# felipescoelho/w-ofdm-optimization

Measured on AMD Instinct MI355X. Metric: OFDM symbols/sec (whole node) + BER vs reference, N=256 16-QAM, higher is better.
Workload: dtype f32

## Files before the change

### w-ofdm-optimization_amd/csrc/wofdm_abi.hip

```cpp
#include "../../include/wofdm.h"
#include "wofdm_kernel.h"

#include <algorithm>
#include <cmath>
#include <complex>
#include <cstdarg>
#include <cstdio>
#include <cstdlib>
#include <cstring>
#include <mutex>
#include <utility>
#include <vector>

namespace {

thread_local char g_err[512] = "";
thread_local float g_papr_ms = 0.f;
thread_local float g_rxprof_ms = 0.f;

int fail(int code, const char *fmt, ...)
{
    va_list ap;
    va_start(ap, fmt);
    vsnprintf(g_err, sizeof g_err, fmt, ap);
// ... 28 lines not shown
        return fail(WOFDM_E_UNSUPPORTED, "n_taps=%d not in [1,%d]", c->n_taps, WOFDM_MAX_TAPS);
    if (c->cp < 0 || c->cs < 0 || c->tail_tx < 0 || c->tail_rx < 0 || (c->tail_rx & 1) ||
        c->prefix_rm < 0 || c->circ_shift < 0 || c->circ_shift >= N)
        return fail(WOFDM_E_INVALID, "negative length, odd tail_rx or circ_shift >= n_fft");
    if (c->cp > N || c->cs > N || c->tail_rx > N)
        return fail(WOFDM_E_INVALID, "cp, cs and tail_rx must not exceed n_fft");
    if (c->n_channels < 1 || c->n_snr < 1 || c->n_window_pairs < 1)
        return fail(WOFDM_E_INVALID, "n_channels, n_snr, n_window_pairs must be >= 1");
    g->N = N; g->k = c->bits_per_sc; g->S = c->syms_per_frame;
    g->mu = c->cp; g->rho = c->cs; g->beta = c->tail_tx; g->delta = c->tail_rx;
    g->gamma = c->prefix_rm; g->kappa = c->circ_shift; g->L = c->n_taps;
    g->P = N + g->mu + g->rho; g->B = g->P - g->beta; g->T = g->beta + g->S * g->B;
    g->NL = c->noise_before_truncate ? g->T + g->L - 1 : g->S * g->B;
    if (2 * g->beta > g->P) return fail(WOFDM_E_INVALID, "2*tail_tx exceeds the symbol length");
    if (g->B != N + g->delta + g->gamma)
        return fail(WOFDM_E_INVALID, "n_fft+cp+cs-tail_tx (%d) != n_fft+tail_rx+prefix_rm (%d)",
                    g->B, N + g->delta + g->gamma);
    if (g->mu + g->rho > wofdm_cpcs_max(N) || g->beta > 16 || g->delta > 64)
        return fail(WOFDM_E_UNSUPPORTED, "kernel limits: cp+cs <= %d, tail_tx <= 16, tail_rx <= 64",
                    wofdm_cpcs_max(N));
    if (g->B > 64 * wofdm_rb(N))
        return fail(WOFDM_E_UNSUPPORTED, "cp+cs-tail_tx=%d exceeds the 64 samples the kernel's "
                    "FIR tiling allows", g->B - N);
    const uint64_t cells = (uint64_t)c->n_channels * c->n_snr * c->n_window_pairs;
    if (cells >= (1u << 28)) return fail(WOFDM_E_UNSUPPORTED, "more than 2^28 cells");
    return WOFDM_OK;
}

}

struct wofdm_plan {
    int device = 0;
    wofdm_cfg cfg{};
    geom g{};
    uint32_t n_cells = 0;
    float *d_wtx = nullptr, *d_wrx = nullptr, *d_nlin = nullptr;
    float2 *d_h = nullptr;
    int *d_geo = nullptr;
    float2 *d_nscr = nullptr;
    uint64_t nscr_elems = 0;
    wofdm_kparams base{};
    wofdm_kernel_fn fn[4] = {nullptr, nullptr, nullptr, nullptr};
    int var = WOFDM_VAR_PLAIN;
    bool has_alloc = false, has_mask = false;
    bool force_direct_mask = false;
    bool fir_valu = false;
    bool dft_valu = false;
    int max_spw = 0;
    uint32_t *d_amask = nullptr;
    float2 *d_tmask = nullptr;
    float2 *d_tspec = nullptr;
    float *d_tspec4 = nullptr;
    unsigned *d_status = nullptr;
    uint4 *d_fira = nullptr;
    float firm_sx = 1.f, firm_sh = 1.f;
    uint4 *d_dftc = nullptr;
    float *d_rxs = nullptr;
#ifdef WOFDM_AUDIT
    uint32_t *audit = nullptr;
    uint32_t audit_items = 0;
#endif
    int occ = 1, cus = 1, layout = 1;
    hipEvent_t ev0 = nullptr, ev1 = nullptr;
};

namespace {

size_t wofdm_amask_words(int N)
{
    const size_t NQ = (size_t)N / 4;
    return N == 256 ? 2 * NQ + 256 : NQ + (NQ > 256 ? NQ : 256);
}

int configure(wofdm_plan *pl)
{
    const geom &g = pl->g;
    const bool fft_ok = g.N <= WOFDM_TXFFT_MAX_N && 3 * g.P - 2 <= WOFDM_TXFFT_LEN && !pl->force_direct_mask;
    const int var = pl->has_mask ? (fft_ok ? WOFDM_VAR_TXFFT : WOFDM_VAR_TXMASK)
                                 : (pl->has_alloc ? WOFDM_VAR_ALLOC : WOFDM_VAR_PLAIN);
    const bool masked = var == WOFDM_VAR_TXMASK || var == WOFDM_VAR_TXFFT;
    const bool firm = !pl->fir_valu;
    const bool mdft = !pl->dft_valu;
    int layout = masked ? wofdm_pick_layout_masked(g.N, g.B, firm) : wofdm_pick_layout(g.N, g.S, g.B, true, firm, mdft);
    if (var == WOFDM_VAR_TXFFT && g.N == 256 && layout == 9 && mdft && WOFDM_TXFFT_LEN == 1024) layout = 15;
    if (pl->max_spw > 0 && wofdm_layout_info(layout, g.N).spw > pl->max_spw)
        layout = (pl->max_spw == 1) ? 1 : wofdm_pick_layout(g.N, g.S, g.B, false);
#ifndef WOFDM_DEV_LDS_PAD
#define WOFDM_DEV_LDS_PAD 0
#endif
    const auto lds_of = [&](int lay) {
        return wofdm_lds_bytes(g.N, g.T, lay, g.S, g.B)
               + (var == WOFDM_VAR_TXMASK ? wofdm_txmask_lds_bytes(g.N) : 0u)
               + (var == WOFDM_VAR_TXFFT && lay != 15 ? wofdm_txfft_lds_bytes() : 0u) + (unsigned)(WOFDM_DEV_LDS_PAD);
    };
    if (!masked && layout != 1 && wofdm_layout_info(layout, g.N).fir == WOFDM_FIR_ONE && lds_of(layout) > 160u * 1024u
        && lds_of(1) <= 160u * 1024u)
        layout = 1;
    const unsigned lds = lds_of(layout);
    if (lds > 160u * 1024u)
        return fail(WOFDM_E_UNSUPPORTED, "frame needs %u bytes of LDS (160 KiB per workgroup)", lds);
    wofdm_kernel_fn fn[4];
    for (int m = 0; m < 4; ++m) {
        fn[m] = wofdm_select_kernel(g.N, g.k, layout, m, var);
        if (!fn[m])
            return fail(WOFDM_E_UNSUPPORTED, "no kernel for n_fft=%d bits_per_sc=%d variant %d%s", g.N, g.k,
                        var, masked ? " (the Tx mask needs n_fft <= 512)" : "");
// ... 53 lines not shown
        const double ang = M_PI * (double)(((long long)k * k) % (2LL * L)) / (double)L;
        c[(size_t)k] = cplx(std::cos(ang), std::sin(ang));
    }
    for (int k = 0; k < L; ++k) a[(size_t)k] = (double)mask[k] * c[(size_t)k];
    b[0] = std::conj(c[0]);
    for (int k = 1; k < L; ++k) b[(size_t)k] = b[Mb - (size_t)k] = std::conj(c[(size_t)k]);
    fft_pow2(a, -1);
    fft_pow2(b, -1);
    for (size_t i = 0; i < Mb; ++i) a[i] *= b[i];
    fft_pow2(a, +1);
    std::vector<cplx> g((size_t)L);
    for (int n = 0; n < L; ++n) g[(size_t)n] = a[(size_t)n] * c[(size_t)n] / ((double)Mb * (double)L);
    return g;
}

void mask_fastconv_spectrum(const float *mask, int L, int MF, float2 *spec)
{
    const int P = (L + 1) / 2, G = 3 * P - 2;
    const std::vector<cplx> g = idft_any(mask, L);
    std::vector<cplx> gt((size_t)MF, cplx(0.0, 0.0));
    for (int t = 0; t < G && t < MF; ++t) gt[(size_t)t] = g[(size_t)(((t - (P - 1)) % L + L) % L)];
    fft_pow2(gt, -1);
    for (int f = 0; f < MF; ++f)
        spec[f] = make_float2((float)(gt[(size_t)f].real() / MF), (float)(gt[(size_t)f].imag() / MF));
}

std::mutex g_gate_mu;
hipEvent_t g_gate_last[64] = {};

int launch(wofdm_plan *pl, int mode, wofdm_kparams &kp, uint64_t total_items, int force_grid,
           hipStream_t stream)
{
    wofdm_kernel_fn fn = pl->fn[mode];
    if (!fn) return fail(WOFDM_E_UNSUPPORTED, "no kernel for n_fft=%d", pl->g.N);
    if (total_items == 0) return WOFDM_OK;
    uint64_t grid = (uint64_t)pl->cus * (uint64_t)pl->occ;
#ifdef WOFDM_DEV_OCC
    grid = (uint64_t)pl->cus * (uint64_t)(WOFDM_DEV_OCC);
#endif
    if (grid > total_items) grid = total_items;
    if (force_grid > 0) grid = (uint64_t)force_grid;
    const size_t row = wofdm_noise_scratch_len(pl->g.N, pl->layout);
    if (row && grid * row > pl->nscr_elems) {
        HIP_TRY(hipDeviceSynchronize());
        if (pl->d_nscr) (void)hipFree(pl->d_nscr);
        pl->d_nscr = nullptr; pl->nscr_elems = 0;
        HIP_TRY(hipMalloc(&pl->d_nscr, grid * row * sizeof(float2)));
        pl->nscr_elems = grid * row;
    }
    kp.noise_scratch = pl->d_nscr;
    kp.status = pl->d_status;
    kp.dftc = pl->d_dftc;
    kp.rx_scale = pl->d_rxs;
    kp.items_q = total_items / grid;
    kp.items_r = total_items % grid;
    kp.lds_bytes = pl->base.lds_bytes;
    float2 *tm = pl->var == WOFDM_VAR_TXFFT ? (pl->layout == 15 ? reinterpret_cast<float2 *>(pl->d_tspec4) : pl->d_tspec) : pl->d_tmask;
    kp.tx_scale = pl->base.tx_scale;
    kp.dump_unscale_tx = pl->base.dump_unscale_tx;
    kp.dump_unscale_rx = pl->base.dump_unscale_rx;
#ifdef WOFDM_AUDIT
    kp.audit = pl->audit; kp.audit_items = pl->audit_items;
#endif
#ifdef WOFDM_DELAY
    {
        const char *dp = std::getenv("WOFDM_DELAY_POINT"), *dw = std::getenv("WOFDM_DELAY_WAVES"), *dn = std::getenv("WOFDM_DELAY_LEN");
        kp.delay_point = dp ? (uint32_t)std::strtoul(dp, nullptr, 0) : 0;
        kp.delay_waves = dw ? (uint32_t)std::strtoul(dw, nullptr, 0) : 0;
        kp.delay_len = dn ? (uint32_t)std::strtoul(dn, nullptr, 0) : 8;
    }
#endif
    void *args[] = {&kp, &pl->d_wtx, &pl->d_wrx, &pl->d_h, &pl->d_nlin, &pl->d_geo, &pl->d_amask, &tm,
                    &pl->d_fira};
    {
        std::lock_guard<std::mutex> lock(g_gate_mu);
        hipEvent_t *last = g_gate_last;
        const int dev = pl->device & 63;
        if (last[dev]) HIP_TRY(hipStreamWaitEvent(stream, last[dev], 0));
        else HIP_TRY(hipEventCreateWithFlags(&last[dev], hipEventDisableTiming));
        HIP_TRY(hipLaunchKernel(reinterpret_cast<const void *>(fn), dim3((unsigned)grid),
                                dim3(64u * (unsigned)wofdm_waves(pl->layout, pl->g.N, pl->g.S, pl->g.B)), args, kp.lds_bytes, stream));
        HIP_TRY(hipEventRecord(last[dev], stream));
    }
    return WOFDM_OK;
}

int check_status(wofdm_plan *pl)
{
    unsigned st = 0;
    HIP_TRY(hipMemcpy(&st, pl->d_status, sizeof st, hipMemcpyDeviceToHost));
    if (st != 0)
        return fail(WOFDM_E_HIP, "kernel status 0x%x: a wave timed out waiting for its workgroup "
                    "(results must not be used)", st);
    return WOFDM_OK;
}

int check_launch_args(wofdm_plan *pl, uint64_t frames_per_cell)
{
    if (!pl) return fail(WOFDM_E_INVALID, "plan is NULL");
    if (frames_per_cell > (1ull << 40)) return fail(WOFDM_E_INVALID, "frames_per_cell too large");
    return WOFDM_OK;
}


template <typename T> struct dev_buf {
    T *p = nullptr;
    dev_buf() = default;
    dev_buf(dev_buf &&o) noexcept : p(o.p) { o.p = nullptr; }
    ~dev_buf() { if (p) (void)hipFree(p); }
    bool alloc(size_t count) { return hipMalloc(&p, count * sizeof(T)) == hipSuccess; }
    bool upload(const void *host, size_t count) { return hipMemcpy(p, host, count * sizeof(T), hipMemcpyHostToDevice) == hipSuccess; }
    operator T *() const { return p; }
};

int use_device(int device)
{
    int ndev = 0;
    HIP_TRY(hipGetDeviceCount(&ndev));
    if (device < 0 || device >= ndev)
        return fail(WOFDM_E_HIP, "device %d not available (%d visible); there is no CPU fallback", device, ndev);
    HIP_TRY(hipSetDevice(device));
    return WOFDM_OK;
}

std::vector<float2> pack_taps(const wofdm_cfg *cfg, const geom &g, const float *h)
{
    std::vector<float2> hp((size_t)cfg->n_channels * WOFDM_LT, make_float2(0.f, 0.f));
    for (int c = 0; c < cfg->n_channels; ++c)
        for (int l = 0; l < g.L; ++l)
            hp[(size_t)c * WOFDM_LT + l] = make_float2(h[2 * ((size_t)c * g.L + l)], h[2 * ((size_t)c * g.L + l) + 1]);
    return hp;
}
// ... 134 lines not shown
            const double rms = (double)pl->firm_sx * (double)pl->firm_sh * std::sqrt(e * (1.0 + (double)nlin[i]) / (double)g.N)
                               * std::fmax(wmax, 1e-30);
            if (rms > 0.0 && std::isfinite(rms))
                rxs[(size_t)i * cfg->n_channels + c] = (float)std::exp2(std::round(4.0 - std::log2(rms)));
        }

#define PLAN_TRY(expr)                                                                        \
    do {                                                                                      \
        hipError_t e_ = (expr);                                                               \
        if (e_ != hipSuccess) {                                                               \
            wofdm_plan_destroy(pl);                                                           \
            return fail(e_ == hipErrorOutOfMemory ? WOFDM_E_NOMEM : WOFDM_E_HIP, "%s: %s",    \
                        #expr, hipGetErrorString(e_));                                        \
        }                                                                                     \
    } while (0)

    PLAN_TRY(hipMalloc(&pl->d_wtx, n_wtx * sizeof(float)));
    PLAN_TRY(hipMalloc(&pl->d_wrx, n_wrx * sizeof(float)));
    PLAN_TRY(hipMalloc(&pl->d_h, hp.size() * sizeof(float2)));
    PLAN_TRY(hipMalloc(&pl->d_nlin, nlin.size() * sizeof(float)));
    PLAN_TRY(hipMemcpy(pl->d_wtx, w_tx, n_wtx * sizeof(float), hipMemcpyHostToDevice));
    PLAN_TRY(hipMemcpy(pl->d_wrx, w_rx, n_wrx * sizeof(float), hipMemcpyHostToDevice));
    PLAN_TRY(hipMemcpy(pl->d_h, hp.data(), hp.size() * sizeof(float2), hipMemcpyHostToDevice));
    PLAN_TRY(hipMemcpy(pl->d_nlin, nlin.data(), nlin.size() * sizeof(float), hipMemcpyHostToDevice));
    PLAN_TRY(hipMalloc(&pl->d_fira, fira.size() * sizeof(_Float16)));
    PLAN_TRY(hipMemcpy(pl->d_fira, fira.data(), fira.size() * sizeof(_Float16), hipMemcpyHostToDevice));
    PLAN_TRY(hipMalloc(&pl->d_dftc, dftc.size() * sizeof(uint32_t)));
    PLAN_TRY(hipMemcpy(pl->d_dftc, dftc.data(), dftc.size() * sizeof(uint32_t), hipMemcpyHostToDevice));
    PLAN_TRY(hipMalloc(&pl->d_rxs, rxs.size() * sizeof(float)));
    PLAN_TRY(hipMemcpy(pl->d_rxs, rxs.data(), rxs.size() * sizeof(float), hipMemcpyHostToDevice));
    PLAN_TRY(hipEventCreate(&pl->ev0));
    PLAN_TRY(hipEventCreate(&pl->ev1));

    int geo[WOFDM_G_COUNT];
    geo[WOFDM_G_S] = g.S; geo[WOFDM_G_MU] = g.mu; geo[WOFDM_G_RHO] = g.rho; geo[WOFDM_G_BETA] = g.beta;
    geo[WOFDM_G_DELTA] = g.delta; geo[WOFDM_G_GAMMA] = g.gamma; geo[WOFDM_G_KAPPA] = g.kappa;
    geo[WOFDM_G_L] = g.L; geo[WOFDM_G_P] = g.P; geo[WOFDM_G_B] = g.B; geo[WOFDM_G_T] = g.T;
    geo[WOFDM_G_NL] = g.NL; geo[WOFDM_G_NSNR] = cfg->n_snr; geo[WOFDM_G_NCH] = cfg->n_channels;
    geo[WOFDM_G_FBUF] = 0;
    geo[WOFDM_G_NACT] = g.N;
    geo[WOFDM_G_SPWR] = 0;
    PLAN_TRY(hipMalloc(&pl->d_geo, sizeof geo));
    PLAN_TRY(hipMemcpy(pl->d_geo, geo, sizeof geo, hipMemcpyHostToDevice));

    wofdm_kparams &kp = pl->base;
    kp.n_cells = pl->n_cells; kp.first_cell = 0; kp.inject_base_cell = 0;
    kp.seed_lo = (uint32_t)cfg->seed; kp.seed_hi = (uint32_t)(cfg->seed >> 32);

    hipDeviceProp_t prop;
    PLAN_TRY(hipGetDeviceProperties(&prop, device));
    pl->cus = prop.multiProcessorCount;
    PLAN_TRY(hipMalloc(&pl->d_status, sizeof(unsigned)));
    PLAN_TRY(hipMemset(pl->d_status, 0, sizeof(unsigned)));
    if ((rc = configure(pl)) != WOFDM_OK) {
        wofdm_plan_destroy(pl);
        return rc;
    }
    const int occ = pl->occ;
    if (const size_t row = wofdm_noise_scratch_len(g.N, pl->layout)) {
        pl->nscr_elems = (uint64_t)pl->cus * (uint64_t)occ * row;
        PLAN_TRY(hipMalloc(&pl->d_nscr, pl->nscr_elems * sizeof(float2)));
        PLAN_TRY(hipMemset(pl->d_nscr, 0, pl->nscr_elems * sizeof(float2)));
        PLAN_TRY(hipDeviceSynchronize());
    }
#undef PLAN_TRY
    *out = pl;
    return WOFDM_OK;
}

int wofdm_plan_destroy(wofdm_plan *pl)
{
    if (!pl) return WOFDM_OK;
    (void)hipSetDevice(pl->device);
    if (pl->d_wtx) (void)hipFree(pl->d_wtx);
    if (pl->d_wrx) (void)hipFree(pl->d_wrx);
    if (pl->d_h) (void)hipFree(pl->d_h);
    if (pl->d_nlin) (void)hipFree(pl->d_nlin);
    if (pl->d_geo) (void)hipFree(pl->d_geo);
    if (pl->d_nscr) (void)hipFree(pl->d_nscr);
    if (pl->d_amask) (void)hipFree(pl->d_amask);
    if (pl->d_tmask) (void)hipFree(pl->d_tmask);
    if (pl->d_tspec) (void)hipFree(pl->d_tspec);
    if (pl->d_tspec4) (void)hipFree(pl->d_tspec4);
    if (pl->d_status) (void)hipFree(pl->d_status);
    if (pl->d_fira) (void)hipFree(pl->d_fira);
    if (pl->d_dftc) (void)hipFree(pl->d_dftc);
    if (pl->d_rxs) (void)hipFree(pl->d_rxs);
    if (pl->ev0) (void)hipEventDestroy(pl->ev0);
    if (pl->ev1) (void)hipEventDestroy(pl->ev1);
    delete pl;
    return WOFDM_OK;
}

int wofdm_plan_set_allocation(wofdm_plan *pl, const uint8_t *active)
{
    if (!pl) return fail(WOFDM_E_INVALID, "plan is NULL");
    HIP_TRY(hipSetDevice(pl->device));
    HIP_TRY(hipDeviceSynchronize());
    const int N = pl->g.N, NQ = N / 4;
    const size_t amask_words = wofdm_amask_words(N);
    int nact = N;
    if (active) {
        nact = 0;
        std::vector<uint32_t> words(amask_words, 0u);
        for (int n = 0; n < N; ++n) {
            if (active[n]) { ++nact; continue; }
            words[(size_t)(n % NQ)] |= 0x80u << (8 * (n / NQ));
            if (N == 256) {
                const int l = n & 15, t = n >> 4;
                words[(size_t)(NQ + 16 * (t & 3) + l)] |= 0x80u << (8 * (t >> 2));
            }
            if (N <= 128) {
                const int sc = N / 16, scs = sc / 4;
                for (int t = 0; t < 4; ++t)
                    for (int lane = 0; lane < 64; ++lane)
                        for (int j = 0; j < 4; ++j)
                            if (sc * (lane / 16 + 4 * j) + 4 * (t % scs) + (lane & 3) == n)
                                words[(size_t)(NQ + 64 * t + lane)] |= 0x80u << (8 * j);
            }
            if (N >= 512 || N == 256) {
                const int nc = N >= 512 ? N / 256 : 1, a = n / (N / 16), r = n % (N / 16), b = r / nc, c = r % nc;
                const int lane = 16 * (a & 3) + b, j = a >> 2;
                words[(size_t)((N == 256 ? 2 * NQ : NQ) + lane + 64 * j)] |= 0x80u << (8 * c);
            }
        }
        if (nact == 0) return fail(WOFDM_E_INVALID, "allocation loads no subcarrier");
        if (!pl->d_amask) HIP_TRY(hipMalloc(&pl->d_amask, amask_words * sizeof(uint32_t)));
        HIP_TRY(hipMemcpy(pl->d_amask, words.data(), amask_words * sizeof(uint32_t), hipMemcpyHostToDevice));
    }
    if (!active && pl->d_amask) HIP_TRY(hipMemset(pl->d_amask, 0, amask_words * sizeof(uint32_t)));
    HIP_TRY(hipMemcpy(pl->d_geo + WOFDM_G_NACT, &nact, sizeof(int), hipMemcpyHostToDevice));
    pl->has_alloc = active && nact < N;
    return configure(pl);
}

int wofdm_plan_set_tx_mask(wofdm_plan *pl, const float *mask)
{
// ... 856 lines not shown
```

### w-ofdm-optimization_amd/csrc/wofdm_kernel.h

```cpp
#pragma once
#include <hip/hip_runtime.h>
#include <stdint.h>

#define WOFDM_LT 21

struct wofdm_kdump {
    uint8_t *labels_tx;
    float2  *X, *tx, *conv, *rx, *Y, *Xhat;
    uint8_t *labels_rx;
    float   *gain;
    float2  *unit_noise;
    float2  *sink;
};

template <int N, bool NOTW = false> struct wofdm_lds {
    static constexpr int TAIL_MAX = 16, CPCS_MAX = N >= 1024 ? 64 : 128, TAILRX_MAX = 64;
    static constexpr int off_tw = 0;
    static constexpr int TW_BYTES = NOTW ? 0 : (N == 256 || N == 512 ? 6 * 64 * 16 : 8 * N);
    static constexpr int off_g = off_tw + TW_BYTES;
    static constexpr int off_sums = off_g + 8 * N;
    static constexpr int off_flags = off_sums + 4 * 64;
    static constexpr int off_wtx = off_flags + 4 * 64;
    static constexpr int off_wrx = off_wtx + 4 * (N + CPCS_MAX);
    static constexpr int off_lut = off_wrx + 4 * (N + TAILRX_MAX);
    static constexpr int off_fbuf = off_lut + 8 * 64;
};

enum { WOFDM_G_S, WOFDM_G_MU, WOFDM_G_RHO, WOFDM_G_BETA, WOFDM_G_DELTA, WOFDM_G_GAMMA, WOFDM_G_KAPPA,
       WOFDM_G_L, WOFDM_G_P, WOFDM_G_B, WOFDM_G_T, WOFDM_G_NL, WOFDM_G_NSNR, WOFDM_G_NCH, WOFDM_G_FBUF,
       WOFDM_G_NACT,
       WOFDM_G_SPWR,
       WOFDM_G_COUNT };

struct wofdm_kparams {
    uint32_t n_cells;
    uint32_t first_cell;
    uint32_t inject_base_cell;
    unsigned lds_bytes;
    uint64_t frames_per_cell, frame_offset;
    uint64_t items_q, items_r;
    uint32_t seed_lo, seed_hi;
    unsigned long long *counts;
    const uint4 *dftc;
    const float *rx_scale;
    const uint8_t *labels;
    const float2  *unit_noise;
    float2 *noise_scratch;
    unsigned *status;
    float tx_scale, dump_unscale_tx, dump_unscale_rx;
    wofdm_kdump dump;
#ifdef WOFDM_DELAY
    uint32_t delay_point, delay_waves, delay_len;
#endif
#ifdef WOFDM_AUDIT
    uint32_t *audit;
    uint32_t audit_items;
#endif
};

#ifndef WOFDM_NOISE_SCRATCH_MIN_N
#define WOFDM_NOISE_SCRATCH_MIN_N 1024
#endif
static inline int wofdm_cpcs_max(int n_fft) { return n_fft >= 1024 ? 64 : 128; }
static inline int wofdm_kslot(int k) { return k == 6 ? 8 : k; }
static constexpr int wofdm_fir8_tiles(int n_fft) { return n_fft >= 1024 ? 9 : (n_fft >= 512 ? 5 : 3); }

enum { WOFDM_FIR_VALU, WOFDM_FIR_QUARTER, WOFDM_FIR_ONE };
enum { WOFDM_DFT_VALU, WOFDM_DFT_MDFT, WOFDM_DFT_BIG, WOFDM_DFT_SMALL };
struct wofdm_layout {
    int spw;
    int fir, dft;
    bool partial;
    bool masked;
    int nt;
    int rb;
    int wg, min_waves;
    int n_min, n_max;
    unsigned vars;
};
#define WOFDM_LAYOUT_COUNT 17
static constexpr wofdm_layout wofdm_layout_info(int id, int n_fft)
{
    const int f8 = wofdm_fir8_tiles(n_fft), sm = 1024 / n_fft;
    const unsigned PA = 3u, MASKS = 12u;
    switch (id) {
    case 1:  return {1,  WOFDM_FIR_VALU,    WOFDM_DFT_VALU,  false, false, 0,  n_fft / 64 + 1,      1024,  4,    64, 1024,  PA | MASKS};
    case 2:  return {2,  WOFDM_FIR_VALU,    WOFDM_DFT_VALU,  false, false, 0,  2 * (n_fft / 64) + 2, 512,  4,    64, 256,   PA};
    case 4:  return {4,  WOFDM_FIR_VALU,    WOFDM_DFT_VALU,  false, false, 0,  4 * (n_fft / 64) + 2, 256,  3,    256, 256,  PA};
    case 5:  return {4,  WOFDM_FIR_VALU,    WOFDM_DFT_VALU,  false, false, 0,  20,                  256,   3,    256, 256,  PA};
    case 6:  return {4,  WOFDM_FIR_QUARTER, WOFDM_DFT_VALU,  false, false, 9,  18,                  256,   3,    256, 256,  PA};
    case 7:  return {4,  WOFDM_FIR_QUARTER, WOFDM_DFT_VALU,  false, false, 10, 20,                  256,   3,    256, 256,  PA};
    case 8:  return {1,  WOFDM_FIR_ONE,     WOFDM_DFT_VALU,  false, false, f8, 2 * f8,              1024,  4,    512, 1024, PA};
    case 9:  return {1,  WOFDM_FIR_ONE,     WOFDM_DFT_VALU,  false, true,  f8, 2 * f8,              1024,  4,    64, 1024,  MASKS};
    case 10: return {4,  WOFDM_FIR_QUARTER, WOFDM_DFT_MDFT,  false, false, 9,  18,                  256,   3,    256, 256,  PA};
    case 11: return {4,  WOFDM_FIR_QUARTER, WOFDM_DFT_MDFT,  false, false, 10, 20,                  256,   3,    256, 256,  PA};
    case 12: return {1,  WOFDM_FIR_ONE,     WOFDM_DFT_BIG,   false, false, f8, 2 * f8,              1024,  4,    512, 1024, PA};
    case 13: return {sm, WOFDM_FIR_QUARTER, WOFDM_DFT_SMALL, false, false, 10, 20,                  n_fft, 3,    64, 128,   PA};
    case 14: return {sm, WOFDM_FIR_QUARTER, WOFDM_DFT_SMALL, false, false, 11, 22,                  n_fft, 3,    64, 128,   PA};
    case 15: return {1,  WOFDM_FIR_ONE,     WOFDM_DFT_BIG,   false, true,  f8, 2 * f8,              1024,  4,    256, 256,  8u};
    case 16: return {sm, WOFDM_FIR_QUARTER, WOFDM_DFT_SMALL, true,  false, 10, 20,                  256,   3,    64, 128,   PA};
    }
    return {};
}
#define WOFDM_FIR8_VT 48
#define WOFDM_FIRM_PRE 24
static inline int wofdm_rb(int n_fft, int layout = 1) { return wofdm_layout_info(layout, n_fft).rb; }
static inline int wofdm_small_spwr(int n_fft, int S, int B)
{
    const int slots = 1024 / n_fft;
    for (int W = 1; W <= 4; ++W) {
        const int spwr = ((S + W - 1) / W + 1) & ~1;
// ... 216 lines not shown
```

### w-ofdm-optimization_amd/csrc/wofdm_kernel.hip

```cpp
#include "wofdm_kernel.h"
#include "wofdm_device.h"
#include "philox.h"
#include <type_traits>
#include <utility>

#ifndef WOFDM_FAULT_SKIP_FLAG
#define WOFDM_FAULT_SKIP_FLAG 0
#endif


#define PRIO_LATENCY 2
#define PRIO_TRANSFORM 1
#define PRIO_TILES 0
#define WAVE_PRIO(x) __builtin_amdgcn_s_setprio(x)

namespace {

#ifdef WOFDM_STAMP
#define STAMP(slot)                                                                            \
    do {                                                                                       \
        __builtin_amdgcn_sched_barrier(0);                                                     \
        const unsigned long long now_ = __builtin_amdgcn_s_memtime();                          \
        __builtin_amdgcn_s_waitcnt(0xC07F);                                                    \
        stamp_acc[slot] += now_ - stamp_t;                                                     \
// ... 452 lines not shown
    constexpr bool FIR8M = LI.masked;
    constexpr bool FIRQ = LI.fir == WOFDM_FIR_QUARTER, FIR8 = LI.fir == WOFDM_FIR_ONE, FIRM = FIRQ || FIR8;
    constexpr int SPW = LI.spw;
    constexpr int NT = LI.nt, PRE = WOFDM_FIRM_PRE;
    constexpr int VT = WOFDM_FIR8_VT;
    constexpr bool ALLOC = VAR >= 1, TXMASK = VAR == 2, TXFFT = VAR == 3;
    constexpr bool RELAX = !DUMP && VAR < 2;
    constexpr bool RELAXM = !DUMP && VAR >= 2;
    constexpr bool RELAXF = RELAX || RELAXM;
    static_assert(!(TXMASK || TXFFT) || SPW == 1, "the Tx mask stage runs one symbol per wave");
    constexpr int LT = WOFDM_LT;
    constexpr int BPL = geo<N>::BPL, NQ = geo<N>::NQ;
    constexpr bool FULL = geo<N>::FULL;
    constexpr bool QW = SPW == 4 && !MDFT && !MDS;
    constexpr int VS = QW ? 1 : (MDS ? 1 : SPW), VB = QW ? 4 : BPL;
    constexpr int RB = fir_geo<N, LAY>::RB, NBK = fir_geo<N, LAY>::NBK;
    constexpr bool EVEN = fir_geo<N, LAY>::EVEN;
    constexpr bool RENOISE = N >= WOFDM_NOISE_SCRATCH_MIN_N;
    constexpr bool RELAUNDER = N >= 1024 || (N >= 512 && VAR >= 2);
    constexpr int LW_MIN = FIR8 ? N : 0;
    extern __shared__ __attribute__((aligned(16))) unsigned char smem[];

    const int tid = threadIdx.x, lane0 = tid & 63;
    const int wv = __builtin_amdgcn_readfirstlane(tid >> 6);
    const int SPWR = PART ? __builtin_amdgcn_readfirstlane(gm[WOFDM_G_SPWR]) : SPW, SPWR2 = SPWR >> 1;
    (void)SPWR2;
    const int s0 = wv * SPWR;
    int lane = lane0;
#define GEO_PHASE()                                                                            \
    int goff_ = 0;                     \
    asm volatile("" : "+s"(goff_));    \
    const int *__restrict__ gq = gm + goff_

    using L = wofdm_lds<N, MDS>;
    v2f *tw = reinterpret_cast<v2f *>(smem + L::off_tw);
    v2f *G = reinterpret_cast<v2f *>(smem + L::off_g);
    float *sums = reinterpret_cast<float *>(smem + L::off_sums);
    lds_vint *flags = (lds_vint *)(smem + L::off_flags);
    float *wtx = reinterpret_cast<float *>(smem + L::off_wtx);
    float *wrx = reinterpret_cast<float *>(smem + L::off_wrx);
    v2f *qlut = reinterpret_cast<v2f *>(smem + L::off_lut);
    v2f *fbuf = reinterpret_cast<v2f *>(smem + L::off_fbuf);
    const v2f *g_h = reinterpret_cast<const v2f *>(g_h_);
    uint32_t *Hp = reinterpret_cast<uint32_t *>(smem + L::off_fbuf);
#define TAILS()                                                                                \
    const int tail_off = gq[WOFDM_G_FBUF];                            \
    v2f *tailb = fbuf + tail_off;                                                                 \
    uint32_t *tH = reinterpret_cast<uint32_t *>(tailb), *tL = tH + gq[WOFDM_G_S] * gq[WOFDM_G_BETA]; \
    (void)tH; (void)tL; (void)tail_off

    DELAY_AT(11);
    for (int i = tid; i < gm[WOFDM_G_FBUF]; i += blockDim.x) fbuf[i] = mk(0.f, 0.f);
    if (tid < 64) flags[tid] = 0;
    if (tid < 64) sums[tid] = 0.f;
    int iter = 0;
    if constexpr (MDS) {
    } else if constexpr (MPIPE) {
        u4 *dl = reinterpret_cast<u4 *>(smem + L::off_tw);
        const u4 *dg = reinterpret_cast<const u4 *>(p.dftc);
        for (int i = tid; i < 6 * 64; i += blockDim.x) dl[i] = dg[i < 256 ? i : i + 256];
    } else if constexpr (QW) fill_twiddles_qw(tw, tid, (int)blockDim.x);
    else fill_twiddles<N>(tw, tid, (int)blockDim.x);
    if (tid < (1 << K)) {
        constexpr int hb = K >> 1, mm = (1 << hb) - 1;
        constexpr float qs = K == 2 ? 0.70710678118654752f : (K == 4 ? 0.31622776601683794f
                                                                     : 0.15430334996209191f);
        const uint32_t gi = (uint32_t)tid >> hb, gq = (uint32_t)tid & (uint32_t)mm;
        const int li = (int)(gi ^ (gi >> 1) ^ (gi >> 2)), lq = (int)(gq ^ (gq >> 1) ^ (gq >> 2));
        if constexpr (MPIPE) {
            const h2 w = {(_Float16)(float)(mm - 2 * lq), (_Float16)(float)(2 * li - mm)};
            reinterpret_cast<uint32_t *>(qlut)[tid] = __builtin_bit_cast(uint32_t, w);
        } else {
            qlut[tid] = mk((float)(2 * li - mm), (float)(mm - 2 * lq)) * qs;
        }
    }
    constexpr float qscale = K == 2 ? 0.70710678118654752f : (K == 4 ? 0.31622776601683794f : 0.15430334996209191f);
    const uint32_t *qlw = reinterpret_cast<const uint32_t *>(qlut);
    (void)qlw;
    v2f *rg = fbuf + gm[WOFDM_G_FBUF] + gm[WOFDM_G_S] * gm[WOFDM_G_BETA];
    if constexpr (TXMASK) {
        const int Lm = 2 * gm[WOFDM_G_P] - 1;
        for (int t = tid; t < mask_geo<N>::RG_LEN; t += blockDim.x) {
            int kk = (t - mask_geo<N>::RG_OFF) % Lm;
            if (kk < 0) kk += Lm;
            rg[t] = ldg2(g_tmask + kk);
        }
    }
    v2f *mtw = fbuf + gm[WOFDM_G_FBUF] + gm[WOFDM_G_S] * gm[WOFDM_G_BETA];
    v2f *mscr = mtw + maskfft_geo::MF;
    if constexpr (TXFFT && !MDM) fill_twiddles<maskfft_geo::MF>(mtw, tid, (int)blockDim.x);
    constexpr int MDM_PK = 344;
    v2f *mdm_park = reinterpret_cast<v2f *>(smem + ((L::off_fbuf + 8 * (gm[WOFDM_G_FBUF] + gm[WOFDM_G_S] * gm[WOFDM_G_BETA]) + 15) & ~15));
    (void)mdm_park;
    __syncthreads();
    DELAY_AT(12);

    constexpr int k = K, half = K >> 1, m1 = (1 << half) - 1;
    constexpr uint32_t lmask = (1u << K) - 1u;
    constexpr float qinv = K == 2 ? 1.4142135623730951f : (K == 4 ? 3.1622776601683795f
                                                                   : 6.4807406984078604f);
    constexpr int ks = K == 6 ? 8 : K;
    constexpr int bps = N * ks / 128;
    static_assert(SPW * bps <= 64, "data-bit blocks of a wave must fit one pass");

    const uint64_t F = p.frames_per_cell;
    const uint64_t bq = blockIdx.x;
    const uint64_t item0 = bq * p.items_q + (bq < p.items_r ? bq : p.items_r);
    uint64_t n_items = p.items_q + (bq < p.items_r ? 1u : 0u);
    const uint32_t cell_rel = (uint32_t)(item0 / F);
    uint32_t cell = __builtin_amdgcn_readfirstlane(p.first_cell + cell_rel);
    uint64_t fidx = item0 - (uint64_t)cell_rel * F;
    {
        const uint32_t flo = __builtin_amdgcn_readfirstlane((uint32_t)fidx);
        const uint32_t fhi = __builtin_amdgcn_readfirstlane((uint32_t)(fidx >> 32));
        fidx = ((uint64_t)fhi << 32) | flo;
    }
    const int n_ch = gm[WOFDM_G_NCH], n_snr = gm[WOFDM_G_NSNR];
    int ch = __builtin_amdgcn_readfirstlane((int)(cell % (uint32_t)n_ch));
    int sn = __builtin_amdgcn_readfirstlane((int)((cell / (uint32_t)n_ch) % (uint32_t)n_snr));
    int pair = __builtin_amdgcn_readfirstlane((int)(cell / ((uint32_t)n_ch * (uint32_t)n_snr)));
    auto next_cell = [&]() {
        ++cell;
        if (++ch == n_ch) { ch = 0; if (++sn == n_snr) { sn = 0; ++pair; } }
    };

    const uint32_t seed_lo = __builtin_amdgcn_readfirstlane(p.seed_lo);
    const uint32_t seed_hi = __builtin_amdgcn_readfirstlane(p.seed_hi);
    uint32_t cur_cell = 0xFFFFFFFFu;
    int cur_pair = -1;
    constexpr bool SCALAR_ACC = N >= 512 || MDM;
    uint32_t bit_err = 0, sym_err = 0, nfr = 0;
    float nlin = 0.f;

    auto flush = [&](uint32_t cabs) {
        const uint32_t c = cabs - p.inject_base_cell;
        const unsigned be = SCALAR_ACC ? bit_err : wave_sum_u(bit_err), se = SCALAR_ACC ? sym_err : wave_sum_u(sym_err);
        if (lane == 0) {
            atomicAdd(&p.counts[4 * (size_t)c + 0], (unsigned long long)be);
            atomicAdd(&p.counts[4 * (size_t)c + 2], (unsigned long long)se);
        }
        if (tid == 0) {
            const int S = gm[WOFDM_G_S];
            const int nact = ALLOC ? gm[WOFDM_G_NACT] : N;
            atomicAdd(&p.counts[4 * (size_t)c + 1], (unsigned long long)nfr * (S - 1) * nact * k);
            atomicAdd(&p.counts[4 * (size_t)c + 3], (unsigned long long)nfr * (S - 1) * nact);
        }
        bit_err = 0; sym_err = 0; nfr = 0;
    };

#ifdef WOFDM_STAMP
    unsigned long long stamp_acc[16] = {0, 0, 0, 0, 0, 0, 0, 0, 0, 0, 0, 0, 0, 0, 0, 0};
    unsigned long long stamp_t = __builtin_amdgcn_s_memtime();
#endif
    for (; n_items != 0; --n_items) {
        STAMP(7);
        WAVE_PRIO(PRIO_LATENCY);
        if (cell != cur_cell || nfr == (1u << 14)) {
            if (cur_cell != 0xFFFFFFFFu) flush(cur_cell);
            const bool refill = pair != cur_pair || (MPIPE && cell != cur_cell);
            cur_cell = cell;
            if (refill) {
                __syncthreads();
                const int P = gm[WOFDM_G_P], delta = gm[WOFDM_G_DELTA];
                int t0 = tid;
                asm volatile("" : "+v"(t0));
                const float txs = MPIPE ? p.tx_scale * qscale : p.tx_scale;
                float rxs = 1.0f;
                if constexpr (MPIPE) rxs = p.rx_scale[sn * n_ch + ch];
                for (int i = t0; i < P; i += blockDim.x)
                    wtx[i] = g_wtx[(size_t)pair * P + i] * txs;
                for (int i = t0; i < N + delta; i += blockDim.x)
                    wrx[i] = g_wrx[(size_t)pair * (N + delta) + i] * rxs;
                __syncthreads();
                cur_pair = pair;
            }
            nlin = g_nlin[sn];
        }
        lane = lane0;
        asm volatile("" : "+v"(lane));
        ++iter;
        float *sums_it = sums + 32 * (iter & 1);
        const uint64_t frame = p.frame_offset + fidx;
        const uint32_t f_lo = (uint32_t)frame, f_hi = (uint32_t)(frame >> 32);
        const size_t inj = ((size_t)(cell - p.inject_base_cell) * F + fidx);
        ++nfr;
        DELAY_AT(1);
#ifdef WOFDM_AUDIT
        float aud_g = 0.f, aud_ps = 0.f, aud_pn = 0.f;
#endif

        v2f v[VS][VB][4];
        uint32_t lab[VS][VB];
        f4 yr[4], yi[4];
        (void)yr; (void)yi;
        uint32_t labo[4] = {0u, 0u, 0u, 0u};
        (void)labo;
        auto mdft_tw2 = [&](f4 (&t2r)[NC], f4 (&t2i)[NC]) {
            const u4 *dg = reinterpret_cast<const u4 *>(p.dftc) + lane;
#pragma unroll
            for (int c = 1; c < NC; ++c) {
                t2r[c] = __builtin_bit_cast(f4, dg[(10 + 2 * (c - 1)) * 64]);
                t2i[c] = __builtin_bit_cast(f4, dg[(11 + 2 * (c - 1)) * 64]);
            }
            t2r[0] = t2i[0] = (f4){0.f, 0.f, 0.f, 0.f};
        };
        (void)mdft_tw2;
// ... 2103 lines not shown
                                lev = mk(lvi[r], lvq[r]);
                            } else {
                                xh = cmul(v[u][q][r], G[n]);
                                lev = __builtin_elementwise_fma(
                                    xh, mk(0.5f * qinv, -0.5f * qinv), mk(0.5f * (float)m1, 0.5f * (float)m1));
                            }
                            iw = __builtin_amdgcn_cvt_pk_u8_f32(__builtin_fminf(lev.x, (float)m1), r, iw);
                            qw = __builtin_amdgcn_cvt_pk_u8_f32(__builtin_fminf(lev.y, (float)m1), r, qw);
                            if (DUMP && p.dump.Xhat) p.dump.Xhat[(s - 1) * N + n] = make_float2(xh.x, xh.y);
                        }
                        constexpr uint32_t GM = K == 2 ? 0u : (K == 4 ? 0x05050505u : 0x1B1B1B1Bu);
                        constexpr uint32_t LM = lmask * 0x01010101u;
                        const uint32_t cw = (iw << half) | qw;
                        const uint32_t gw = cw ^ ((cw >> 1) & GM);
                        uint32_t diff = (gw ^ lab[u][q]) & LM;
                        if constexpr (ALLOC) {
                            diff &= ~(((lab[u][q] >> 7) & 0x01010101u) * 0xFFu);
                        }
                        if constexpr (SCALAR_ACC) {
                            be_f += __popc(diff);
                            se_f += __popc((diff + 0x7F7F7F7Fu) & 0x80808080u);
                        } else {
                            bit_err += __popc(diff);
                            sym_err += __popc((diff + 0x7F7F7F7Fu) & 0x80808080u);
                        }
                        if (DUMP && p.dump.labels_rx) {
#pragma unroll
                            for (int r = 0; r < 4; ++r)
                                p.dump.labels_rx[(s - 1) * N + sub_of(q, r)] = (uint8_t)((gw >> (8 * r)) & lmask);
                        }
                    }
                }
            }
        }

        if constexpr (SCALAR_ACC) {
            bit_err += wave_sum_u(be_f);
            sym_err += wave_sum_u(se_f);
#ifdef WOFDM_AUDIT
            if (p.audit && (uint32_t)(iter - 1) < p.audit_items) {
                const unsigned ab = wave_sum_u(be_f), as = wave_sum_u(se_f);
                if (lane == 0) {
                    uint32_t *a = p.audit + (((size_t)blockIdx.x * p.audit_items + (uint32_t)(iter - 1)) * 16 + wv) * 8;
                    a[0] = ab; a[1] = as; a[2] = __float_as_uint(aud_g); a[3] = __float_as_uint(aud_ps);
                    a[4] = __float_as_uint(aud_pn); a[5] = __builtin_amdgcn_s_getreg(4 | (31 << 11));
                    a[6] = __builtin_amdgcn_s_getreg(20 | (31 << 11)); a[7] = (uint32_t)__builtin_amdgcn_s_memtime();
                }
            }
#endif
        }
        STAMP(6);
        if (++fidx == F) { fidx = 0; next_cell(); }
    }
    if (cur_cell != 0xFFFFFFFFu) flush(cur_cell);
    if constexpr (RELAXF) {
        __syncthreads();
        if (tid == 0 && flags[20] != 0) atomicOr(p.status, 1u);
    }
#ifdef WOFDM_STAMP
    if (lane0 == 0) {
        unsigned long long *dst = p.counts + 4 * (size_t)(p.first_cell + p.n_cells)
                                  + ((size_t)blockIdx.x * 16 + wv) * 16;
        for (int i = 0; i < 16; ++i) dst[i] = stamp_acc[i];
    }
#endif
}

template <int N, int K, int LAY, int VAR> wofdm_kernel_fn pick_mode(int mode)
{
    if constexpr (wofdm_layout_built(LAY, N, VAR)) {
        switch (mode) {
        case WOFDM_MODE_GEN: return wofdm_frames_kernel<N, K, LAY, false, false, VAR>;
        case WOFDM_MODE_INJECT: return wofdm_frames_kernel<N, K, LAY, true, false, VAR>;
        case WOFDM_MODE_DUMP_GEN: return wofdm_frames_kernel<N, K, LAY, false, true, VAR>;
        case WOFDM_MODE_DUMP_INJECT: return wofdm_frames_kernel<N, K, LAY, true, true, VAR>;
        }
    }
    return nullptr;
}

template <int N, int K, int LAY> wofdm_kernel_fn pick_var(int mode, int var)
{
    switch (var) {
    case WOFDM_VAR_PLAIN: return pick_mode<N, K, LAY, WOFDM_VAR_PLAIN>(mode);
    case WOFDM_VAR_ALLOC: return pick_mode<N, K, LAY, WOFDM_VAR_ALLOC>(mode);
    case WOFDM_VAR_TXMASK: return pick_mode<N, K, LAY, WOFDM_VAR_TXMASK>(mode);
    case WOFDM_VAR_TXFFT: return pick_mode<N, K, LAY, WOFDM_VAR_TXFFT>(mode);
    }
    return nullptr;
}

template <int N, int K, int... LAYS>
wofdm_kernel_fn pick_layout(int layout, int mode, int var, std::integer_sequence<int, LAYS...>)
{
    wofdm_kernel_fn fn = nullptr;
    ((layout == LAYS ? (void)(fn = pick_var<N, K, LAYS>(mode, var)) : (void)0), ...);
    return fn;
}

template <int N> wofdm_kernel_fn pick(int k, int layout, int mode, int var)
{
    if (k != WOFDM_TU_K) return nullptr;
    return pick_layout<N, WOFDM_TU_K>(layout, mode, var, std::make_integer_sequence<int, WOFDM_LAYOUT_COUNT>{});
}

}
// ... 12 lines not shown
```

Measured before the change: 1.095 billion.

## Add dynamic work-stealing tail split across workgroups via global atomic counter

Replaces the static per-block item partition with a hybrid split. Each workgroup gets a fixed head share (a fraction alpha of its even share), and the remaining items are handed out in small chunks through a global atomic counter that is reset before each launch. The aim is to even out per-block imbalance and the straggler tail across CUs when occupancy is at least 2 and there are many items per block. The cost is atomics and extra block barriers per chunk, plus a memset per launch; the scheme is gated to certain layouts and can be tuned through environment variables.

```diff
diff --git a/w-ofdm-optimization_amd/csrc/wofdm_abi.hip b/w-ofdm-optimization_amd/csrc/wofdm_abi.hip
--- a/w-ofdm-optimization_amd/csrc/wofdm_abi.hip
+++ b/w-ofdm-optimization_amd/csrc/wofdm_abi.hip
@@ -104,6 +104,9 @@
     float2 *d_tspec = nullptr;
     float *d_tspec4 = nullptr;
     unsigned *d_status = nullptr;
+    unsigned long long *d_work = nullptr;
+    uint32_t split_alpha_256 = WOFDM_SPLIT_ALPHA_256, split_chunk = WOFDM_SPLIT_CHUNK;
+    bool split_forced = false;
     uint4 *d_fira = nullptr;
     float firm_sx = 1.f, firm_sh = 1.f;
     uint4 *d_dftc = nullptr;
@@ -263,8 +266,12 @@
     kp.status = pl->d_status;
     kp.dftc = pl->d_dftc;
     kp.rx_scale = pl->d_rxs;
-    kp.items_q = total_items / grid;
-    kp.items_r = total_items % grid;
+    const bool dynamic = (mode == WOFDM_MODE_GEN || mode == WOFDM_MODE_INJECT) && wofdm_layout_dynamic(pl->layout, pl->g.N)
+                         && (pl->split_forced || (pl->occ >= 2 && total_items / grid >= WOFDM_SPLIT_MIN_ITEMS));
+    const wofdm_split sp = wofdm_work_split(total_items, grid, dynamic, pl->split_alpha_256, pl->split_chunk);
+    kp.head_q = sp.head_q; kp.head_r = sp.head_r; kp.tail0 = sp.tail0; kp.total = total_items;
+    kp.chunk = sp.chunk;
+    kp.work = pl->d_work;
     kp.lds_bytes = pl->base.lds_bytes;
     float2 *tm = pl->var == WOFDM_VAR_TXFFT ? (pl->layout == 15 ? reinterpret_cast<float2 *>(pl->d_tspec4) : pl->d_tspec) : pl->d_tmask;
     kp.tx_scale = pl->base.tx_scale;
@@ -289,6 +296,7 @@
         const int dev = pl->device & 63;
         if (last[dev]) HIP_TRY(hipStreamWaitEvent(stream, last[dev], 0));
         else HIP_TRY(hipEventCreateWithFlags(&last[dev], hipEventDisableTiming));
+        if (kp.tail0 < kp.total) HIP_TRY(hipMemsetAsync(pl->d_work, 0, sizeof(unsigned long long), stream));
         HIP_TRY(hipLaunchKernel(reinterpret_cast<const void *>(fn), dim3((unsigned)grid),
                                 dim3(64u * (unsigned)wofdm_waves(pl->layout, pl->g.N, pl->g.S, pl->g.B)), args, kp.lds_bytes, stream));
         HIP_TRY(hipEventRecord(last[dev], stream));
@@ -529,6 +537,26 @@
     pl->cus = prop.multiProcessorCount;
     PLAN_TRY(hipMalloc(&pl->d_status, sizeof(unsigned)));
     PLAN_TRY(hipMemset(pl->d_status, 0, sizeof(unsigned)));
+    PLAN_TRY(hipMalloc(&pl->d_work, sizeof(unsigned long long)));
+    PLAN_TRY(hipMemset(pl->d_work, 0, sizeof(unsigned long long)));
+    if (const char *e = std::getenv("WOFDM_SPLIT_ALPHA")) {
+        const double a = std::strtod(e, nullptr);
+        if (!(a >= 0.0 && a < 1.0)) {
+            wofdm_plan_destroy(pl);
+            return fail(WOFDM_E_INVALID, "WOFDM_SPLIT_ALPHA=%s: a fraction in [0, 1)", e);
+        }
+        pl->split_alpha_256 = (uint32_t)(a * 256.0);
+        pl->split_forced = true;
+    }
+    if (const char *e = std::getenv("WOFDM_SPLIT_CHUNK")) {
+        const unsigned long c = std::strtoul(e, nullptr, 0);
+        if (c < 1 || c > (1ul << 20)) {
+            wofdm_plan_destroy(pl);
+            return fail(WOFDM_E_INVALID, "WOFDM_SPLIT_CHUNK=%s: 1 ... 2^20 items", e);
+        }
+        pl->split_chunk = (uint32_t)c;
+        pl->split_forced = true;
+    }
     if ((rc = configure(pl)) != WOFDM_OK) {
         wofdm_plan_destroy(pl);
         return rc;
@@ -560,6 +588,7 @@
     if (pl->d_tspec) (void)hipFree(pl->d_tspec);
     if (pl->d_tspec4) (void)hipFree(pl->d_tspec4);
     if (pl->d_status) (void)hipFree(pl->d_status);
+    if (pl->d_work) (void)hipFree(pl->d_work);
     if (pl->d_fira) (void)hipFree(pl->d_fira);
     if (pl->d_dftc) (void)hipFree(pl->d_dftc);
     if (pl->d_rxs) (void)hipFree(pl->d_rxs);
diff --git a/w-ofdm-optimization_amd/csrc/wofdm_kernel.h b/w-ofdm-optimization_amd/csrc/wofdm_kernel.h
--- a/w-ofdm-optimization_amd/csrc/wofdm_kernel.h
+++ b/w-ofdm-optimization_amd/csrc/wofdm_kernel.h
@@ -38,7 +38,9 @@
     uint32_t inject_base_cell;
     unsigned lds_bytes;
     uint64_t frames_per_cell, frame_offset;
-    uint64_t items_q, items_r;
+    uint64_t head_q, head_r, tail0, total;
+    uint32_t chunk;
+    unsigned long long *work;
     uint32_t seed_lo, seed_hi;
     unsigned long long *counts;
     const uint4 *dftc;
@@ -57,6 +59,22 @@
     uint32_t audit_items;
 #endif
 };
+
+static constexpr bool wofdm_layout_dynamic(int layout, int n_fft)
+{
+    return layout == 10 || layout == 11 || layout == 13 || layout == 14 || layout == 16 || (layout == 12 && n_fft == 512);
+}
+#define WOFDM_SPLIT_ALPHA_256 192
+#define WOFDM_SPLIT_CHUNK 8
+#define WOFDM_SPLIT_MIN_ITEMS 512
+struct wofdm_split { uint64_t head_q, head_r, tail0; uint32_t chunk; };
+static inline wofdm_split wofdm_work_split(uint64_t total, uint64_t grid, bool dynamic, uint32_t alpha_256, uint32_t chunk)
+{
+    const uint64_t q = total / grid;
+    if (!dynamic || total <= grid) return {q, total % grid, total, 0u};
+    const uint64_t head = (q >> 8) * alpha_256 + (((q & 255u) * alpha_256) >> 8);
+    return {head, 0u, head * grid, chunk};
+}
 
 #ifndef WOFDM_NOISE_SCRATCH_MIN_N
 #define WOFDM_NOISE_SCRATCH_MIN_N 1024
diff --git a/w-ofdm-optimization_amd/csrc/wofdm_kernel.hip b/w-ofdm-optimization_amd/csrc/wofdm_kernel.hip
--- a/w-ofdm-optimization_amd/csrc/wofdm_kernel.hip
+++ b/w-ofdm-optimization_amd/csrc/wofdm_kernel.hip
@@ -528,6 +528,21 @@
     DELAY_AT(11);
     for (int i = tid; i < gm[WOFDM_G_FBUF]; i += blockDim.x) fbuf[i] = mk(0.f, 0.f);
     if (tid < 64) flags[tid] = 0;
+    enum { WS_OFF_LO = 17, WS_OFF_HI = 18,
+           WS_CHUNK = 19,
+           WS_LEFT_LO = 21, WS_LEFT_HI = 22,
+           WS_TAIL0_LO = 23, WS_TAIL0_HI = 28,
+           WS_WORK_LO = 29, WS_WORK_HI = 30,
+           WS_CELL0 = 31 };
+    constexpr bool DYN = !DUMP && wofdm_layout_dynamic(LAY, N);
+    if (DYN && tid == 0) {
+        const uint64_t left = p.total - p.tail0, wp = (uint64_t)(uintptr_t)p.work;
+        flags[WS_CHUNK] = (int)p.chunk;
+        flags[WS_LEFT_LO] = (int)(uint32_t)left; flags[WS_LEFT_HI] = (int)(uint32_t)(left >> 32);
+        flags[WS_TAIL0_LO] = (int)(uint32_t)p.tail0; flags[WS_TAIL0_HI] = (int)(uint32_t)(p.tail0 >> 32);
+        flags[WS_WORK_LO] = (int)(uint32_t)wp; flags[WS_WORK_HI] = (int)(uint32_t)(wp >> 32);
+        flags[WS_CELL0] = (int)p.first_cell;
+    }
     if (tid < 64) sums[tid] = 0.f;
     int iter = 0;
     if constexpr (MDS) {
@@ -580,24 +595,48 @@
     static_assert(SPW * bps <= 64, "data-bit blocks of a wave must fit one pass");
 
     const uint64_t F = p.frames_per_cell;
-    const uint64_t bq = blockIdx.x;
-    const uint64_t item0 = bq * p.items_q + (bq < p.items_r ? bq : p.items_r);
-    uint64_t n_items = p.items_q + (bq < p.items_r ? 1u : 0u);
-    const uint32_t cell_rel = (uint32_t)(item0 / F);
-    uint32_t cell = __builtin_amdgcn_readfirstlane(p.first_cell + cell_rel);
-    uint64_t fidx = item0 - (uint64_t)cell_rel * F;
-    {
+    const int n_ch = gm[WOFDM_G_NCH], n_snr = gm[WOFDM_G_NSNR];
+    uint64_t n_items = p.head_q + (blockIdx.x < p.head_r ? 1u : 0u), fidx = 0;
+    uint32_t cell = 0;
+    int ch = 0, sn = 0, pair = 0;
+    auto ws_get = [&](int i) { return __builtin_amdgcn_readfirstlane((uint32_t)flags[i]); };
+    auto ws_get64 = [&](int lo, int hi) { return ((uint64_t)ws_get(hi) << 32) | ws_get(lo); };
+    auto seek = [&](uint64_t item, uint32_t first_cell) {
+        uint32_t f_lo = (uint32_t)F, f_hi = (uint32_t)(F >> 32);
+        uint32_t nc = (uint32_t)n_ch, ns = (uint32_t)n_snr;
+        if constexpr (DYN) asm volatile("" : "+s"(f_lo), "+s"(f_hi), "+s"(nc), "+s"(ns));
+        const uint64_t Fd = ((uint64_t)f_hi << 32) | f_lo;
+        const uint32_t cell_rel = (uint32_t)(item / Fd);
+        cell = __builtin_amdgcn_readfirstlane(first_cell + cell_rel);
+        fidx = item - (uint64_t)cell_rel * Fd;
         const uint32_t flo = __builtin_amdgcn_readfirstlane((uint32_t)fidx);
         const uint32_t fhi = __builtin_amdgcn_readfirstlane((uint32_t)(fidx >> 32));
         fidx = ((uint64_t)fhi << 32) | flo;
-    }
-    const int n_ch = gm[WOFDM_G_NCH], n_snr = gm[WOFDM_G_NSNR];
-    int ch = __builtin_amdgcn_readfirstlane((int)(cell % (uint32_t)n_ch));
-    int sn = __builtin_amdgcn_readfirstlane((int)((cell / (uint32_t)n_ch) % (uint32_t)n_snr));
-    int pair = __builtin_amdgcn_readfirstlane((int)(cell / ((uint32_t)n_ch * (uint32_t)n_snr)));
+        ch = __builtin_amdgcn_readfirstlane((int)(cell % nc));
+        sn = __builtin_amdgcn_readfirstlane((int)((cell / nc) % ns));
+        pair = __builtin_amdgcn_readfirstlane((int)(cell / (nc * ns)));
+    };
+    uint64_t item = (uint64_t)blockIdx.x * p.head_q + (blockIdx.x < p.head_r ? blockIdx.x : p.head_r);
     auto next_cell = [&]() {
         ++cell;
         if (++ch == n_ch) { ch = 0; if (++sn == n_snr) { sn = 0; ++pair; } }
+    };
+    auto take_chunk = [&](uint32_t chunk) {
+        if (tid == 0) {
+            typedef __attribute__((address_space(1))) unsigned long long gu64;
+            gu64 *work = (gu64 *)(((uint64_t)(uint32_t)flags[WS_WORK_HI] << 32) | (uint32_t)flags[WS_WORK_LO]);
+            const unsigned long long off = __hip_atomic_fetch_add(work, (unsigned long long)chunk, __ATOMIC_RELAXED, __HIP_MEMORY_SCOPE_AGENT);
+            flags[WS_OFF_LO] = (int)(uint32_t)off;
+            flags[WS_OFF_HI] = (int)(uint32_t)(off >> 32);
+        }
+        __syncthreads();
+        const uint64_t off = ws_get64(WS_OFF_LO, WS_OFF_HI);
+        __syncthreads();
+        const uint64_t left = ws_get64(WS_LEFT_LO, WS_LEFT_HI);
+        if (off >= left) return false;
+        n_items = left - off < (uint64_t)chunk ? left - off : (uint64_t)chunk;
+        item = ws_get64(WS_TAIL0_LO, WS_TAIL0_HI) + off;
+        return true;
     };
 
     const uint32_t seed_lo = __builtin_amdgcn_readfirstlane(p.seed_lo);
@@ -628,6 +667,8 @@
     unsigned long long stamp_acc[16] = {0, 0, 0, 0, 0, 0, 0, 0, 0, 0, 0, 0, 0, 0, 0, 0};
     unsigned long long stamp_t = __builtin_amdgcn_s_memtime();
 #endif
+    for (;;) {
+    if constexpr (DYN) seek(item, ws_get(WS_CELL0)); else seek(item, p.first_cell);
     for (; n_items != 0; --n_items) {
         STAMP(7);
         WAVE_PRIO(PRIO_LATENCY);
@@ -2837,6 +2878,14 @@
         STAMP(6);
         if (++fidx == F) { fidx = 0; next_cell(); }
     }
+#ifdef WOFDM_STAMP
+    STAMP(7);
+#endif
+    if constexpr (DYN) {
+        const uint32_t chunk = ws_get(WS_CHUNK);
+        if (chunk == 0 || !take_chunk(chunk)) break;
+    } else break;
+    }
     if (cur_cell != 0xFFFFFFFFu) flush(cur_cell);
     if constexpr (RELAXF) {
         __syncthreads();
```

After: 1.196 billion (median of 6 runs). +9.2%, better.
